# ironmanaudi/GNN-decode

Hardware: NVIDIA B200
Metric: decoded syndromes/sec (higher is better)
Workload: dtype f32

## Files before the change

### gnn_decode_b200/csrc/gd_lean.cu

```cuda
#include "gd_lean.cuh"
#include "gd_decode.cuh"
#include "gd_math.cuh"
#include "gd_options.cuh"
#include <algorithm>
#include <cmath>
#include <stddef.h>
#include <string.h>

namespace gd {

constexpr uint32_t kNone = 0xFFFFFFFFu;
constexpr int kMaxSlots = kLeanMaxSlots;
constexpr int kHdrBytes = 2048;
constexpr float kBudgetC = 1e-7f;
constexpr float kBudgetV = 1e-6f;
constexpr float kBudgetR = 4e-6f;

static_assert(sizeof(LeanHeader) <= kHdrBytes, "header");

struct LeanParams {
    const int* idx;
    const uint32_t* sgn;
    float* prob; float* logit; uint8_t* hard; uint32_t* hard_bits;
    LeanHeader* hdr;
    LeanCall* call;
    LeanCall* next_call;
    float* stash;
    LeanTrainHdr* train;
    const int* idx_src;
    const float4* ctab; const float4* rtab; const float4* vtab;
    const uint32_t* meta;
    long long B;
    int T, V, C, E, nw, vw, P;
    int v_lo, nv, part;
    int R, G, NCH;
    int ct_n, rt_n, vt_n;
    int train_vt_max;
    int off_me, off_ms, off_mi, off_var, off_ct, off_rt, off_vt, off_state;
};

__device__ __forceinline__ uint32_t lds_u32(uint32_t a) {
    uint32_t v;
    asm("ld.shared.u32 %0, [%1];" : "=r"(v) : "r"(a));
    return v;
}
__device__ __forceinline__ uint4 lds_u128(uint32_t a) {
    uint4 v;
    asm("ld.shared.v4.u32 {%0,%1,%2,%3}, [%4];" : "=r"(v.x), "=r"(v.y), "=r"(v.z), "=r"(v.w) : "r"(a));
    return v;
}
__device__ __forceinline__ uint2 lds_u64(uint32_t a) {
    uint2 v;
    asm("ld.shared.v2.u32 {%0,%1}, [%2];" : "=r"(v.x), "=r"(v.y) : "r"(a));
    return v;
}
__device__ __forceinline__ float4 lds_f128(uint32_t a) {
    float4 v;
    asm("ld.shared.v4.f32 {%0,%1,%2,%3}, [%4];" : "=f"(v.x), "=f"(v.y), "=f"(v.z), "=f"(v.w) : "r"(a));
    return v;
}
template <int OFF>
__device__ __forceinline__ float lds_state(uint32_t a) {
    float v;
    asm volatile("ld.shared.f32 %0, [%1+%2];" : "=f"(v) : "r"(a), "n"(OFF));
    return v;
}
template <int OFF>
__device__ __forceinline__ void sts_state(uint32_t a, float v) {
    asm volatile("st.shared.f32 [%0+%1], %2;" ::"r"(a), "n"(OFF), "f"(v));
}
__device__ __forceinline__ float lds_state_rt(uint32_t a) {
    float v;
    asm volatile("ld.shared.f32 %0, [%1];" : "=f"(v) : "r"(a));
    return v;
}
__device__ __forceinline__ void sts_state_rt(uint32_t a, float v) { asm volatile("st.shared.f32 [%0], %1;" ::"r"(a), "f"(v)); }
__device__ __forceinline__ void group_bar(int id, int nthreads) {
    asm volatile("bar.sync %0, %1;" ::"r"(id), "r"(nthreads) : "memory");
}

template <int STRIDE>
__device__ __forceinline__ float lean_cubic(uint32_t base, float w) {
    const float v = w + 12582912.0f;
    const float tau = w - (v - 12582912.0f);
    const float4 c = lds_f128((uint32_t)__float_as_int(v) * (uint32_t)STRIDE + base);
    return fmaf(fmaf(fmaf(c.w, tau, c.z), tau, c.y), tau, c.x);
}
template <int STRIDE>
__device__ __forceinline__ uint32_t lean_base(uint32_t piece0) {
    uint32_t b = piece0 - 0x4B400000u * (uint32_t)STRIDE;
    asm volatile("" : "+r"(b));
    return b;
}

__device__ __forceinline__ float lean_cubic_rt(uint32_t base, float w, uint32_t stride) {
    const float v = w + 12582912.0f;
    const float tau = w - (v - 12582912.0f);
    const float4 c = lds_f128((uint32_t)__float_as_int(v) * stride + base);
    return fmaf(fmaf(fmaf(c.w, tau, c.z), tau, c.y), tau, c.x);
}

struct LeanTabs {
    uint32_t vt_stride;
    uint32_t vt_base;
    uint32_t ct_base;
    float vt_inv_h, vt_off;
    float ct_inv_h, ct_off;
    float t0;
};

__device__ __forceinline__ float lean_vt(const LeanTabs& tb, float m) {
    return lean_cubic_rt(tb.vt_base, fmaf(m, tb.vt_inv_h, tb.vt_off), tb.vt_stride);
}
__device__ __forceinline__ float lean_ct(const LeanTabs& tb, float ext) {
    return lean_cubic<128>(tb.ct_base, fmaf(ext, tb.ct_inv_h, tb.ct_off));
}

template <int DEG, int NSIB, int CUR, int NXT, bool STASH>
__device__ __forceinline__ void lean_check(const uint4 eo, const uint4 so, uint32_t st_lane, const LeanTabs& tb, uint32_t sgn,
                                           float* stash_q, long long Bp) {
    const uint32_t eoa[4] = {eo.x, eo.y, eo.z, eo.w}, soa[4] = {so.x, so.y, so.z, so.w};
    float t[4], mo[4];
#pragma unroll
    for (int j = 0; j < 4; ++j) {
        t[j] = j < NSIB ? lean_vt(tb, lds_state<CUR>(st_lane + soa[j])) : (j < DEG ? tb.t0 : 0.f);
        mo[j] = j < DEG ? lds_state<CUR>(st_lane + eoa[j]) : 0.f;
    }
    const float a = t[0] + t[1], b = t[2] + t[3];
    const float ext[4] = {t[1] + b, t[0] + b, a + t[3], a + t[2]};
#pragma unroll
    for (int j = 0; j < DEG; ++j) {
        const float o = lean_ct(tb, ext[j]);
        const float mn = mo[j] + __uint_as_float(__float_as_uint(o) ^ sgn);
        sts_state<NXT>(st_lane + eoa[j], mn);
        if (STASH && stash_q) stash_q[(long long)(eoa[j] >> 8) * Bp] = mn;
    }
}

template <int CUR, bool STASH>
__device__ __forceinline__ void lean_iteration(const LeanParams& p, uint32_t me, uint32_t ms, uint32_t mi, uint32_t st_lane,
                                               const LeanTabs& tb, uint32_t mybits, float* stash_q) {
    constexpr int NXT = 128 - CUR;
#pragma unroll 1
    for (int k = 0; k < p.NCH; ++k) {
        const uint32_t kind = lds_u32(mi + 4u * k) & 63u;
        if (kind == 0) break;
        const uint4 eo = lds_u128(me + 16u * k), so = lds_u128(ms + 16u * k);
        const uint32_t sgn = (mybits >> k) << 31;
        switch (kind) {
#define GD_LEAN_CASE(D, S) case ((D) | ((S) << 3)): lean_check<D, S, CUR, NXT, STASH>(eo, so, st_lane, tb, sgn, stash_q, p.B); break;
            GD_LEAN_CASE(4, 4) GD_LEAN_CASE(4, 3) GD_LEAN_CASE(4, 2) GD_LEAN_CASE(4, 1) GD_LEAN_CASE(4, 0)
            GD_LEAN_CASE(3, 3) GD_LEAN_CASE(3, 2) GD_LEAN_CASE(3, 1) GD_LEAN_CASE(3, 0)
            GD_LEAN_CASE(2, 2) GD_LEAN_CASE(2, 1) GD_LEAN_CASE(2, 0)
            GD_LEAN_CASE(1, 1) GD_LEAN_CASE(1, 0)
#undef GD_LEAN_CASE
            default: break;
        }
    }
}

__device__ __forceinline__ void lean_deal(int n_slots, const int* counts, int* out4, int lane) {
        const int grid = (int)gridDim.x;
        int tl[2], nc[2];
        int total = 0;
#pragma unroll
        for (int h = 0; h < 2; ++h) {
            const int k = lane + 32 * h;
            tl[h] = k < n_slots ? (counts[k] + 31) >> 5 : 0;
            total += tl[h];
        }
        for (int o = 16; o > 0; o >>= 1) total += __shfl_xor_sync(0xffffffffu, total, o);
        int given = 0;
#pragma unroll
        for (int h = 0; h < 2; ++h) {
            nc[h] = tl[h] ? max(1, (int)((long long)grid * tl[h] / max(total, 1))) : 0;
            given += nc[h];
        }
        for (int o = 16; o > 0; o >>= 1) given += __shfl_xor_sync(0xffffffffu, given, o);
        for (int left = grid - given; left != 0; left += left > 0 ? -1 : 1) {
            float best = -3e38f;
            int who = -1;
#pragma unroll
            for (int h = 0; h < 2; ++h) {
                const bool can = left > 0 ? tl[h] > 0 : nc[h] > 1;
                const float load = left > 0 ? (float)tl[h] / (float)max(nc[h], 1) : -(float)tl[h] / (float)max(nc[h] - 1, 1);
                if (can && load > best) { best = load; who = lane + 32 * h; }
            }
            for (int o = 16; o > 0; o >>= 1) {
                const float ob = __shfl_xor_sync(0xffffffffu, best, o);
                const int ow = __shfl_xor_sync(0xffffffffu, who, o);
                if (ow >= 0 && (who < 0 || ob > best || (ob == best && ow < who))) { best = ob; who = ow; }
            }
            if (who < 0) break;
#pragma unroll
            for (int h = 0; h < 2; ++h)
                if (who == lane + 32 * h) nc[h] += left > 0 ? 1 : -1;
        }
        int my_slot = -1, my_part = 0, my_n = 1, my_tiles = 0, my_row0 = 0;
        int cta_acc = 0, row_acc = 0;
        for (int k = 0; k < n_slots; ++k) {
            const int src = k & 31, h = k >> 5;
            const int nk = __shfl_sync(0xffffffffu, h ? nc[1] : nc[0], src), tk = __shfl_sync(0xffffffffu, h ? tl[1] : tl[0], src);
            if (my_slot < 0 && nk > 0 && (int)blockIdx.x >= cta_acc && (int)blockIdx.x < cta_acc + nk) {
                my_slot = k; my_part = (int)blockIdx.x - cta_acc; my_n = nk; my_tiles = tk; my_row0 = row_acc;
            }
            cta_acc += nk;
            row_acc += counts[k];
        }
        if (lane == 0) {
            out4[0] = my_slot;
            out4[1] = my_slot >= 0 ? (int)((long long)my_part * my_tiles / my_n) : 0;
            out4[2] = my_slot >= 0 ? (int)((long long)(my_part + 1) * my_tiles / my_n) : 0;
            out4[3] = my_row0;
        }
}

template <bool STASH>
__global__ void __launch_bounds__(1024, 1) lean_decode_kernel(const LeanParams p) {
    extern __shared__ __align__(128) unsigned char smem[];
    __shared__ int tile_pre[4];
    pdl_enter();
    const LeanHeader* H = p.hdr;
    const int tid = threadIdx.x, lane = tid & 31, warp = tid >> 5;
    if (blockIdx.x == 0) {
        if (tid == 0) { p.next_call->overflow = 0; p.next_call->defer_count = 0; p.next_call->fmax_new = 0u; p.next_call->d2_new = 0u; p.next_call->d3_new = 0u; }
        if (tid < kMaxSlots) p.next_call->count[tid] = 0;
    }
    const int n_slots = H->n_slots;
    const float fmax = __uint_as_float(H->fmax_bits), f3max = __uint_as_float(H->f3max_bits);
    const bool overflow = p.call->overflow != 0;
    const int vt_n = H->vt_n_eff, vt_rep = vt_n > 0 ? (8 * p.vt_n) / vt_n : 0;
    const int vt_n_max = STASH ? p.train_vt_max : 8 * p.vt_n;
    bool ok = !overflow && n_slots <= kMaxSlots && vt_n >= p.vt_n && vt_n <= vt_n_max && __uint_as_float(H->err_c_bits) <= kBudgetC + 6e-8f * fmax &&
              __uint_as_float(H->err_r_bits) <= kBudgetR + 1e-7f * f3max && isfinite(fmax) && isfinite(f3max);
    const float gain = 6.0f * (float)p.T * __uint_as_float(H->d2max_bits) * __uint_as_float(H->d3max_bits);
    const float budget_v = gain > 400.0f ? 4e-4f / gain : kBudgetV;
    bool ok_v = isfinite(gain);
    float worst_v = 0.f;
    for (int k = 0; k < n_slots && k < kMaxSlots; ++k)
        if (p.call->count[k] != 0) worst_v = fmaxf(worst_v, __uint_as_float(H->err_v_bits[k]));
    ok_v = ok_v && worst_v <= budget_v;
    if (blockIdx.x == 0 && tid == 0 && ok && !overflow) {
        const int mult = max(1, H->vt_mult);
        if (!ok_v && vt_n < vt_n_max) { p.hdr->vt_mult = 2 * vt_n / p.vt_n; p.hdr->hash = 0ull; p.hdr->forced = 1; }
        else if (ok_v && mult > 1 && vt_n == mult * p.vt_n && worst_v * 32.0f < budget_v) p.hdr->vt_mult = mult / 2;
    }
    ok = ok && ok_v;
    if (STASH) ok = ok && p.call->defer_count == 0;
    if (STASH && blockIdx.x == 0 && tid < kMaxSlots) {
        if (tid == 0) {
            p.train->status = ok ? 1 : 0;
            p.train->old_count = ok ? 0 : -1;
            p.train->n_slots = n_slots;
            p.train->fmax_bits = H->fmax_bits;
            p.train->vt_n_eff = vt_n;
        }
        p.train->count[tid] = tid < n_slots ? p.call->count[tid] : 0;
        p.train->slot_bits[tid] = H->slot_bits[tid];
    }
    if (blockIdx.x == 0 && tid == 0) {
        if (overflow) {
            p.hdr->n_slots = 0;
            p.hdr->built_mask = 0ull;
            for (int k = 0; k < kMaxSlots; ++k) { p.hdr->slot_bits[k] = kNone; p.hdr->err_v_bits[k] = 0u; }
        } else {
            p.hdr->built_mask = n_slots >= 64 ? ~0ull : ((1ull << n_slots) - 1ull);
        }
        if (!ok) p.call->defer_count = -1;
    }
    if (!ok) return;
    if (n_slots == 0) return;
    if (STASH) {
        int* dst = reinterpret_cast<int*>(reinterpret_cast<float*>(p.train) + kLeanTrainTailFloats);
        for (long long i = (long long)blockIdx.x * blockDim.x + tid; i < p.B; i += (long long)gridDim.x * blockDim.x) dst[i] = p.idx_src[i];
    }

    if (warp == 0) lean_deal(n_slots, p.call->count, tile_pre, lane);
    __syncthreads();
    const int k = tile_pre[0], j_lo = tile_pre[1], j_hi = tile_pre[2];
    if (k < 0 || j_lo >= j_hi) return;
    {
        const uint4* src = reinterpret_cast<const uint4*>(p.meta);
        uint4* dst = reinterpret_cast<uint4*>(smem + p.off_me);
        const int n16 = (p.off_ct - p.off_me) >> 4;
        for (int i = tid; i < n16; i += blockDim.x) dst[i] = src[i];
        float4* ct = reinterpret_cast<float4*>(smem + p.off_ct);
        for (int i = tid; i < (p.ct_n + 2) * 8; i += blockDim.x) ct[i] = __ldg(p.ctab + (i >> 3));
        float4* rt = reinterpret_cast<float4*>(smem + p.off_rt);
        for (int i = tid; i < p.rt_n + 2; i += blockDim.x) rt[i] = __ldg(p.rtab + i);
        float4* vt = reinterpret_cast<float4*>(smem + p.off_vt);
        const float4* vsrc = p.vtab + (size_t)k * (8 * p.vt_n + 2);
        for (int i = tid; i < (vt_n + 2) * vt_rep; i += blockDim.x) vt[i] = __ldg(vsrc + i / vt_rep);
    }
    __syncthreads();
    const int grp = warp / p.R, r = warp - grp * p.R;
    const uint32_t s_base = (uint32_t)__cvta_generic_to_shared(smem);
    const uint32_t me = s_base + p.off_me + (uint32_t)(r * p.NCH) * 16u;
    const uint32_t ms = s_base + p.off_ms + (uint32_t)(r * p.NCH) * 16u;
    const uint32_t mi = s_base + p.off_mi + (uint32_t)(r * p.NCH) * 4u;
    const uint32_t st_lane = s_base + p.off_state + (uint32_t)grp * (uint32_t)p.E * 256u + (uint32_t)lane * 4u;
    const int bar_id = 1 + grp, bar_n = 32 * p.R;
    const float Rm = (float)p.T * (fmax * 1.02f + 1e-6f);
    LeanTabs tb;
    tb.vt_inv_h = 0.5f * (float)vt_n / Rm;
    tb.vt_off = Rm * tb.vt_inv_h - 0.5f;
    tb.ct_inv_h = (float)p.ct_n / 6.0f;
    tb.ct_off = 3.0f * tb.ct_inv_h - 0.5f;
    tb.ct_base = lean_base<128>(s_base + p.off_ct + 128u + (uint32_t)(lane & 7) * 16u);
    tb.vt_stride = 16u * (uint32_t)vt_rep;
    {
        uint32_t b = s_base + p.off_vt + tb.vt_stride + (uint32_t)(lane & (vt_rep - 1)) * 16u - 0x4B400000u * tb.vt_stride;
        asm volatile("" : "+r"(b));
        tb.vt_base = b;
    }
    const float rt_inv_h = 0.5f * (float)p.rt_n / Rm, rt_off = Rm * rt_inv_h - 0.5f;
    const uint32_t rt_base = lean_base<16>(s_base + p.off_rt + 16u);
    const int fin = (p.T & 1) * 128, oth = 128 - fin;

    {
        const float prior = __uint_as_float(H->slot_bits[k]);
        const int cnt = p.call->count[k];
        const int* rows = p.idx + tile_pre[3];
        tb.t0 = lean_vt(tb, 0.f);
        for (int j = j_lo + grp; j < j_hi; j += p.G) {
            const int li = j * 32 + lane;
            const bool live = li < cnt;
            const long long sg = live ? (long long)__ldg(rows + li) : 0;
            float* const stash_q = (STASH && live) ? p.stash + tile_pre[3] + li : nullptr;
            uint32_t mybits = 0;
            for (int q = 0; q < p.NCH; ++q) {
                const uint32_t info = lds_u32(mi + 4u * q);
                if ((info & 7u) == 0) break;
                const int c = (int)(info >> 8);
                const uint32_t wv = live ? __ldg(p.sgn + sg * p.nw + (c >> 5)) : 0u;
                mybits |= ((wv >> (c & 31)) & 1u) << q;
            }
            for (int q = 0; q < p.NCH; ++q) {
                const int deg = (int)(lds_u32(mi + 4u * q) & 7u);
                if (deg == 0) break;
                const uint4 eo = lds_u128(me + 16u * q);
                const float o = lean_ct(tb, (float)(deg - 1) * tb.t0);
                const float mv = __uint_as_float(__float_as_uint(o) ^ ((mybits >> q) << 31));
                const uint32_t eoa[4] = {eo.x, eo.y, eo.z, eo.w};
#pragma unroll
                for (int e = 0; e < 4; ++e)
                    if (e < deg) {
                        sts_state<128>(st_lane + eoa[e], mv);
                        if (STASH && stash_q) stash_q[(long long)(eoa[e] >> 8) * p.B] = mv;
                    }
            }
            group_bar(bar_id, bar_n);
            int it = 1;
            const long long EB = (long long)p.E * p.B;
            for (; it + 1 < p.T; it += 2) {
                lean_iteration<128, STASH>(p, me, ms, mi, st_lane, tb, mybits, stash_q ? stash_q + it * EB : nullptr);
                group_bar(bar_id, bar_n);
                lean_iteration<0, STASH>(p, me, ms, mi, st_lane, tb, mybits, stash_q ? stash_q + (it + 1) * EB : nullptr);
                group_bar(bar_id, bar_n);
            }
            if (it < p.T) {
                lean_iteration<128, STASH>(p, me, ms, mi, st_lane, tb, mybits, stash_q ? stash_q + it * EB : nullptr);
                group_bar(bar_id, bar_n);
            }
            const uint32_t st_grp = st_lane - (uint32_t)lane * 4u;
            for (int v = r; v < p.nv; v += p.R) {
                const uint2 ve = lds_u64(s_base + p.off_var + 8u * v);
                float acc = prior;
                if (ve.x != kNone) acc += lean_cubic<16>(rt_base, fminf(fmaxf(fmaf(lds_state_rt(st_lane + ve.x + fin), rt_inv_h, rt_off), -1.4f), (float)p.rt_n + 0.4f));
                if (ve.y != kNone) acc += lean_cubic<16>(rt_base, fminf(fmaxf(fmaf(lds_state_rt(st_lane + ve.y + fin), rt_inv_h, rt_off), -1.4f), (float)p.rt_n + 0.4f));
                const uint32_t q = (uint32_t)lane * (uint32_t)p.P + (uint32_t)v;
                sts_state_rt(st_grp + (q >> 5) * 256u + (q & 31u) * 4u + oth, acc);
            }
            group_bar(bar_id, bar_n);
            const int nvalid = min(32, cnt - j * 32);
            for (int s = r; s < nvalid; s += p.R) {
                const long long row = __shfl_sync(0xffffffffu, sg, s);
                for (int w = p.v_lo >> 5; w <= (p.v_lo + p.nv - 1) >> 5; ++w) {
                    const int v = w * 32 + lane, vl = v - p.v_lo;
                    const bool mine = vl >= 0 && vl < p.nv;
                    const uint32_t q = (uint32_t)s * (uint32_t)p.P + (uint32_t)(mine ? vl : 0);
                    const float lv = mine ? lds_state_rt(st_grp + (q >> 5) * 256u + (q & 31u) * 4u + oth) : 1.0f;
                    const float pr = sigmoid_neg(lv);
                    if (mine) {
                        if (p.prob) p.prob[row * p.V + v] = pr;
                        if (p.logit) p.logit[row * p.V + v] = lv;
                        if (p.hard) p.hard[row * p.V + v] = pr > 0.5f;
                    }
                    if (p.hard_bits) {
                        const uint32_t word = __ballot_sync(0xffffffffu, mine && pr > 0.5f);
                        if (lane == 0) { if (p.part) atomicOr(p.hard_bits + row * p.vw + w, word); else p.hard_bits[row * p.vw + w] = word; }
                    }
                }
            }
            group_bar(bar_id, bar_n);
        }
    }
}

struct MlpD {
    const float* w1; int w1s; const float* w1b; const float* b1; const float* w2; float b2; int h;
};
__device__ __forceinline__ void mlp_eval_warp(const MlpD& M, double prior, double x, int lane, double& f, double& df) {
    double sf = 0.0, sd = 0.0;
    for (int k = lane; k < M.h; k += 32) {
        const double a = (double)M.w1[k * M.w1s];
        double c = (double)M.b1[k];
        if (M.w1b) c += (double)M.w1b[k * M.w1s] * prior;
        const double z = a * x + c;
        double sp, sg;
        if (z > 20.0) { sp = z; sg = 1.0; }
        else {
            const double e = exp(-fabs(z));
            sp = fmax(z, 0.0) + log1p(e);
            sg = z >= 0.0 ? 1.0 / (1.0 + e) : e / (1.0 + e);
        }
        const double w2 = (double)M.w2[k];
        sf += w2 * sp;
        sd += w2 * a * sg;
    }
    for (int o = 16; o > 0; o >>= 1) {
        sf += __shfl_xor_sync(0xffffffffu, sf, o);
        sd += __shfl_xor_sync(0xffffffffu, sd, o);
    }
    f = sf + (double)M.b2;
    df = sd;
}
__device__ __forceinline__ void atomic_max_float_up(unsigned int* dst, double v) {
    const float f = __double2float_ru(fabs(v));
    atomicMax(dst, __float_as_uint(f));
}

constexpr int kChunk = 32;

__device__ void build_chunk(const MlpD& M, double prior, bool tanh_fold, double Rdom, int n, int i0, int n_int, float4* dst,
                            unsigned int* fmax_bits, unsigned int* dmax_bits, unsigned int* err_bits, double2* nodes ) {
    const int lane = threadIdx.x & 31, warp = threadIdx.x >> 5, nwarp = blockDim.x >> 5;
    const double h = 2.0 * Rdom / (double)n;
    for (int j = warp; j <= n_int; j += nwarp) {
        const double x = -Rdom + h * (double)(i0 - 1 + j);
        double f, df;
        mlp_eval_warp(M, prior, x, lane, f, df);
        if (lane == 0 && fmax_bits) atomic_max_float_up(fmax_bits, f);
        if (lane == 0 && dmax_bits) atomic_max_float_up(dmax_bits, df);
        if (tanh_fold) {
// ... 781 lines not shown
            for (int j = 0; j < 4; ++j) me[4 * i + j] = 0u, ms[4 * i + j] = kNone;
            mi[i] = 0u;
            if (k >= (int)own[r].size()) continue;
            const int c = own[r][k], b = g->h_chk_ptr[c], d = g->h_chk_ptr[c + 1] - b;
            int j = 0, nsib = 0;
            for (int pass = 0; pass < 2; ++pass)
                for (int q = 0; q < d; ++q) {
                    const int e = g->h_chk_edges[b + q];
                    const uint32_t sb = sibling(e);
                    if ((sb != kNone) != (pass == 0)) continue;
                    me[4 * i + j] = (uint32_t)loc[e] * 256u;
                    ms[4 * i + j] = sb;
                    nsib += sb != kNone;
                    ++j;
                }
            mi[i] = (uint32_t)d | ((uint32_t)nsib << 3) | ((uint32_t)c << 8);
        }
    for (int i = 0; i < sub->nv; ++i) {
        const int v = sub->v_lo + i, b = g->h_var_ptr[v], d = g->h_var_ptr[v + 1] - b;
        var[2 * i] = d > 0 ? (uint32_t)loc[g->h_var_edges[b]] * 256u : kNone;
        var[2 * i + 1] = d > 1 ? (uint32_t)loc[g->h_var_edges[b + 1]] * 256u : kNone;
    }
    if (cudaMalloc((void**)&m.dev, m.bytes) != cudaSuccess ||
        cudaMemcpy(m.dev, blob.data(), m.bytes, cudaMemcpyHostToDevice) != cudaSuccess) {
        if (m.dev) cudaFree(m.dev);
        m.dev = nullptr;
        cudaGetLastError();
    }
    ctx->metas.push_back(mp);
    return mp->dev ? mp : nullptr;
}

static bool lean_applicable(const gd_graph* g, const gd_model* m) {
    if (m->program != GD_PROG_V2_4 || m->flags != 0 || m->iters < 1 || m->iters > 32 || opt_on(OPT_NO_LEAN)) return false;
    if (g->max_var_deg > 2 || g->max_chk_deg > 4 || g->E >= (1 << 23) / 256) return false;
    return true;
}

static const int kLeanRts[] = {2048, 1024};
static int lean_rt_choice(gd_graph* g, const std::vector<const LeanSub*>& parts, int ct_n, int vt_n) {
    const int smem_max = g->max_smem_optin - 1024;
    int ri_all = 0;
    for (const LeanSub* sub : parts) {
        int g_cap[2] = {0, 0};
        for (int R = 1; R <= 32; ++R) {
            std::vector<std::vector<int>> own;
            int nch;
            double bal;
            assign_owners(g, sub, R, own, &nch, &bal);
            if (nch > 32 || nch == 0) continue;
            const int meta = align_up_i(align_up_i(2 * R * nch * 16 + R * nch * 4, 16) + sub->nv * 8, 16);
            for (int ri = 0; ri < 2; ++ri) {
                const int fixed = align_up_i(meta + (ct_n + 2) * 128 + (kLeanRts[ri] + 2) * 16 + (vt_n + 2) * 128, 128);
                g_cap[ri] = std::max(g_cap[ri], std::min((smem_max - fixed) / (sub->E * 256), std::min(32 / R, 15)));
            }
        }
        if (g_cap[1] < 1) return -1;
        if (!(g_cap[0] >= std::min(g_cap[1], 3) && g_cap[0] >= 1)) ri_all = 1;
    }
    return ri_all;
}

static bool lean_search(gd_graph* g, const LeanSub* sub, int tpc, int ri_fixed, LeanGeom* out) {
    const int E = sub->E, V = sub->nv;
    const int ct_n = (int)std::min<long long>(1024, std::max<long long>(32, opt_int(OPT_LEAN_CTAB_N, 128)));
    const int vt_n = (int)std::min<long long>(4096, std::max<long long>(64, opt_int(OPT_LEAN_VTAB_N, 512)));
    const int state = E * 256;
    const int smem_max = g->max_smem_optin - 1024;
    struct Cand { int R, G, NCH, rt_n; double score; };
    Cand best{0, 0, 0, 0, -1.0};
    const int* rts = kLeanRts;
    const long long force_R = opt_int(OPT_LEAN_R, 0), force_G = opt_int(OPT_LEAN_G, 0);
    const long long force_rt = opt_int(OPT_LEAN_RTAB_N, 0);
    std::vector<int> nchs(33, 0);
    std::vector<double> bals(33, 0.0);
    for (int R = 1; R <= 32; ++R) {
        std::vector<std::vector<int>> own;
        assign_owners(g, sub, R, own, &nchs[R], &bals[R]);
    }
    for (int R = 1; R <= 32; ++R) {
        if (force_R > 0 && R != force_R) continue;
        const int nch = nchs[R];
        const double bal = bals[R];
        if (nch > 32 || nch == 0) continue;
        const int meta = align_up_i(align_up_i(2 * R * nch * 16 + R * nch * 4, 16) + V * 8, 16);
        for (int ri = ri_fixed; ri <= ri_fixed; ++ri) {
            const int rt_n = force_rt > 0 ? (int)force_rt : rts[ri];
            const int fixed = align_up_i(meta + (ct_n + 2) * 128 + (rt_n + 2) * 16 + (vt_n + 2) * 128, 128);
            int G = (smem_max - fixed) / state;
            G = std::min(G, std::min(32 / R, 15));
            if (force_G > 0) G = G >= force_G ? (int)force_G : 0;
            if (G < 1) continue;
            const int warps = G * R;
            const double eff = (double)tpc / (double)(((tpc + G - 1) / G) * G);
            double score = (warps / (warps + 8.0)) * (G / (G + 0.8)) * std::sqrt(eff) * (0.4 + 0.6 * bal);
            if (score > best.score) best = Cand{R, G, nch, rt_n, score};
        }
    }
    if (best.R > 0 && force_R <= 0) {
        auto max_load = [&](int R) { return bals[R] > 0.0 ? (int)std::lround((double)E / ((double)R * bals[R])) : 0; };
        const int mx0 = max_load(best.R);
        for (int R = best.R + 1; R <= 32 && R * best.G <= 32; ++R) {
            if (nchs[R] == 0 || nchs[R] > best.NCH || max_load(R) > mx0) continue;
            const int meta = align_up_i(align_up_i(2 * R * nchs[R] * 16 + R * nchs[R] * 4, 16) + V * 8, 16);
            const int fixed = align_up_i(meta + (ct_n + 2) * 128 + (best.rt_n + 2) * 16 + (vt_n + 2) * 128, 128);
            if ((smem_max - fixed) / state < best.G) continue;
            best.R = R; best.NCH = nchs[R];
        }
    }
    out->valid = true;
    out->R = best.R; out->G = best.G; out->NCH = best.NCH; out->rt_n = best.rt_n;
    out->ct_n = ct_n; out->vt_n = vt_n;
    return true;
}

static bool lean_fill(gd_graph* g, const LeanSub* sub, const gd_model* m, int64_t B, const LeanGeom& best, const LeanMeta* meta, LeanPlan* out) {
    const int E = sub->E, V = g->V, ct_n = best.ct_n, vt_n = best.vt_n, state = E * 256;
    const int smem_max = g->max_smem_optin;
    LeanParams& p = out->p;
    memset(&p, 0, sizeof(p));
    p.B = B; p.T = m->iters; p.V = V; p.C = g->C; p.E = E;
    p.nw = (g->C + 31) / 32; p.vw = (V + 31) / 32; p.P = sub->nv | 1;
    p.v_lo = sub->v_lo; p.nv = sub->nv; p.part = sub->id >= 0 ? 1 : 0;
    p.R = best.R; p.G = best.G; p.NCH = meta->NCH;
    p.ct_n = ct_n; p.rt_n = best.rt_n; p.vt_n = vt_n;
    p.meta = meta->dev;
    p.off_me = 0; p.off_ms = meta->off_ms; p.off_mi = meta->off_mi; p.off_var = meta->off_var;
    p.off_ct = (int)meta->bytes;
    p.off_rt = p.off_ct + (ct_n + 2) * 128;
    p.off_vt = p.off_rt + (best.rt_n + 2) * 16;
    p.off_state = align_up_i(p.off_vt + (vt_n + 2) * 128, 128);
    out->smem = p.off_state + best.G * state;
    out->threads = 32 * best.G * best.R;
    out->n_tiles = (int)((B + 31) / 32);
    out->grid = g->sm_count;
    out->meta = meta;
    return out->smem <= smem_max - 1024;
}

static bool lean_plan(gd_graph* g, const gd_model* m, int64_t B, std::vector<LeanPlan>* out, bool whole_only = false) {
    out->clear();
    if (!lean_applicable(g, m)) return false;
    const std::vector<LeanSub*>& subs = lean_subs(g);
    const int ct_n = (int)std::min<long long>(1024, std::max<long long>(32, opt_int(OPT_LEAN_CTAB_N, 128)));
    const int vt_n = (int)std::min<long long>(4096, std::max<long long>(64, opt_int(OPT_LEAN_VTAB_N, 512)));
    const int tpc = (int)std::min<long long>(64, std::max<long long>(1, ((B + 31) / 32 + g->sm_count - 1) / g->sm_count));
    LeanCtx* ctx = static_cast<LeanCtx*>(g->lean_ctx);
    int mode = -2, ri = -1;
    {
        std::lock_guard<std::mutex> lk(g->mu);
        if (ctx->mode_epoch == opt_epoch()) { mode = ctx->mode[whole_only ? 1 : 0]; ri = ctx->mode_ri[whole_only ? 1 : 0]; }
    }
    if (mode == -2) {
        int modes[2], ris[2];
        const int ri_whole = (subs[0]->nv | 1) <= subs[0]->E ? lean_rt_choice(g, {subs[0]}, ct_n, vt_n) : -1;
        std::vector<const LeanSub*> comps(subs.begin() + 1, subs.end());
        bool comps_ok = !comps.empty();
        for (const LeanSub* c : comps) comps_ok = comps_ok && (c->nv | 1) <= c->E;
        const int ri_comps = comps_ok ? lean_rt_choice(g, comps, ct_n, vt_n) : -1;
        const long long want = opt_int(OPT_LEAN_PARTS, -1);
        modes[1] = ri_whole >= 0 ? 0 : -1; ris[1] = ri_whole;
        if (ri_comps >= 0 && (ri_whole < 0 || want == 1) && want != 0) { modes[0] = 1; ris[0] = ri_comps; }
        else { modes[0] = modes[1]; ris[0] = ri_whole; }
        std::lock_guard<std::mutex> lk(g->mu);
        ctx->mode_epoch = opt_epoch();
        for (int i = 0; i < 2; ++i) { ctx->mode[i] = modes[i]; ctx->mode_ri[i] = ris[i]; }
        mode = modes[whole_only ? 1 : 0]; ri = ris[whole_only ? 1 : 0];
    }
    if (mode < 0) return false;
    const size_t first = mode == 0 ? 0 : 1, last = mode == 0 ? 1 : subs.size();
    for (size_t si = first; si < last; ++si) {
        const LeanSub* sub = subs[si];
        LeanGeom geom;
        {
            std::lock_guard<std::mutex> lk(g->mu);
            if (!ctx->geoms.empty() && ctx->geoms[0].opt_epoch != opt_epoch()) ctx->geoms.clear();
            for (const LeanGeom& q : ctx->geoms)
                if (q.tpc == tpc && q.sub == sub->id) geom = q;
        }
        if (!geom.valid) {
            if (!lean_search(g, sub, tpc, ri, &geom)) return false;
            geom.opt_epoch = opt_epoch();
            geom.tpc = tpc;
            geom.sub = sub->id;
            std::lock_guard<std::mutex> lk(g->mu);
            if (ctx->geoms.size() >= 128) ctx->geoms.clear();
            ctx->geoms.push_back(geom);
        }
        if (geom.R == 0) return false;
        const LeanMeta* meta = get_meta(g, sub, geom.R);
        if (!meta) return false;
        LeanPlan pl;
        if (!lean_fill(g, sub, m, B, geom, meta, &pl)) return false;
        pl.n_parts = (int)(last - first);
        out->push_back(pl);
    }
    return !out->empty();
}

bool lean_launch_info(const gd_graph* g, const gd_model* model, int64_t B, gd_launch_info* out) {
    std::vector<LeanPlan> pls;
    if (!lean_plan(const_cast<gd_graph*>(g), model, B, &pls)) return false;
    const LeanPlan& pl = pls[0];
    out->tile = 32 * pl.p.G; out->threads = pl.threads; out->grid = pl.grid; out->smem_bytes = pl.smem;
    out->resident = 1; out->n_tiles = (int)pls.size() * ((pl.n_tiles + pl.p.G - 1) / pl.p.G);
    return true;
}

template <typename P>
static cudaError_t pdl_launch(void (*kern)(const P), dim3 grid, dim3 block, size_t smem, cudaStream_t st, const P& params) {
    return pdl_launch_on(!opt_on(OPT_NO_PDL), kern, grid, block, smem, st, params);
}

static cudaMemPool_t lean_pool(gd_graph* g) {
    std::lock_guard<std::mutex> lk(g->mu);
    if (!g->lean_ctx) g->lean_ctx = new LeanCtx();
    LeanCtx* ctx = static_cast<LeanCtx*>(g->lean_ctx);
    if (!ctx->pool) {
        cudaMemPoolProps props;
        memset(&props, 0, sizeof(props));
        props.allocType = cudaMemAllocationTypePinned;
        props.handleTypes = cudaMemHandleTypeNone;
        props.location.type = cudaMemLocationTypeDevice;
        props.location.id = g->device;
        if (cudaMemPoolCreate(&ctx->pool, &props) != cudaSuccess) {
            ctx->pool = nullptr;
            cudaGetLastError();
            return nullptr;
        }
        unsigned long long keep = ~0ull;
        cudaMemPoolSetAttribute(ctx->pool, cudaMemPoolAttrReleaseThreshold, &keep);
    }
    return ctx->pool;
}

static bool lean_bwd_geom(gd_graph* g, const LeanParams& fp, LeanBwdGeom* out) {
    LeanCtx* ctx = static_cast<LeanCtx*>(g->lean_ctx);
    const int tpc = (int)std::min<long long>(64, std::max<long long>(1, ((fp.B + 31) / 32 + g->sm_count - 1) / g->sm_count));
    {
        std::lock_guard<std::mutex> lk(g->mu);
        if (!ctx->bwd.empty() && ctx->bwd[0].opt_epoch != opt_epoch()) ctx->bwd.clear();
        for (const LeanBwdGeom& c : ctx->bwd)
            if (c.valid && c.tpc == tpc && c.ct_n == fp.ct_n && c.rt_n == fp.rt_n && c.vt_n == fp.vt_n) {
                *out = c;
                return c.R > 0;
            }
    }
    const int E = (int)g->E, ct_n = fp.ct_n, rt_n = fp.rt_n, vt_n = fp.vt_n;
    const int smem_max = g->max_smem_optin - 1024;
    auto fixed_bytes = [&](int meta, int n) {
        return align_up_i(meta + (ct_n + 2 + rt_n + 2 + n + 2) * 16 + 16 * (ct_n + 3 + rt_n + 3 + n + 3), 128);
    };
    LeanBwdGeom b;
    double best = -1.0;
    std::vector<int> nchs(33, 0), mxs(33, 0), metas(33, 0);
    auto take = [&](int R, int G) {
        b.R = R; b.G = G;
        b.vt_max = vt_n;
        for (int mult = 2; mult <= 4; mult *= 2)
            if (fixed_bytes(metas[R], mult * vt_n) + 3 * E * 128 <= smem_max) b.vt_max = mult * vt_n;
    };
    for (int R = 1; R <= 32; ++R) {
        std::vector<std::vector<int>> own;
        int nch;
        double bal;
        assign_owners(g, lean_subs(g)[0], R, own, &nch, &bal);
        if (nch == 0 || nch > 32) continue;
        const int meta = align_up_i(align_up_i(2 * R * nch * 16 + R * nch * 4, 16) + g->V * 8, 16);
        nchs[R] = nch; metas[R] = meta; mxs[R] = bal > 0.0 ? (int)std::lround((double)E / ((double)R * bal)) : 0;
        int G = (smem_max - fixed_bytes(meta, vt_n)) / (3 * E * 128);
        G = std::min(G, std::min(32 / R, 15));
        if (G < 1) continue;
        G = std::min(G, tpc);
        const int warps = G * R;
        const double eff = (double)tpc / (double)(((tpc + G - 1) / G) * G);
        const double score = (warps / (warps + 8.0)) * (G / (G + 0.8)) * std::sqrt(eff) * (0.4 + 0.6 * bal);
        if (score > best) { best = score; take(R, G); }
    }
    if (b.R > 0) {
        const int r0 = b.R;
        for (int R = r0 + 1; R <= 32 && R * b.G <= 32; ++R) {
            if (nchs[R] == 0 || nchs[R] > nchs[r0] || mxs[R] > mxs[r0]) continue;
            if ((smem_max - fixed_bytes(metas[R], vt_n)) / (3 * E * 128) < b.G) continue;
            take(R, b.G);
        }
    }
    b.ct_n = ct_n; b.rt_n = rt_n; b.vt_n = vt_n; b.tpc = tpc; b.opt_epoch = opt_epoch(); b.valid = true;
    {
        std::lock_guard<std::mutex> lk(g->mu);
// ... 51 lines not shown
        hit->ct_n = p.ct_n; hit->rt_n = p.rt_n; hit->vt_n = p.vt_n;
    }
    hit->last_use = ++ctx->tick;
    return hit;
}

int lean_decode(gd_graph* g, const gd_model* model, const float* weights_dev, const float* x_dev, const float* prior_dev,
                const uint32_t* synd_dev, float* prob_dev, float* logit_dev, uint8_t* hard_dev, uint32_t* hard_bits_dev,
                int64_t B, cudaStream_t st, float* stash_dev) {
    std::vector<LeanPlan> pls;
    if (!lean_plan(g, model, B, &pls, stash_dev != nullptr)) return -1;
    cudaMemPool_t pool = lean_pool(g);
    if (!pool) return -1;
    LeanCtx* ctx = static_cast<LeanCtx*>(g->lean_ctx);
    std::lock_guard<std::mutex> enq(ctx->enq);
    LeanParams& p = pls[0].p;
    LeanEntry* ent = lean_entry(g, ctx, p, model, weights_dev, st);
    if (!ent) return -1;
    const int N = g->N;
    size_t off = 0;
    auto take = [&](size_t bytes) { const size_t o = off; off = (off + bytes + 255) & ~(size_t)255; return o; };
    const size_t o_slot = take((size_t)B * 2), o_pos = take((size_t)B * 4), o_idx = take((size_t)B * 4);
    const size_t o_sgn = take(x_dev ? (size_t)B * p.nw * 4 : 0);
    const size_t o_defer = take((size_t)B * 4), o_x = take(x_dev ? 0 : (size_t)B * N * 4);
    unsigned char* ws = nullptr;
    GD_CUDA(cudaMallocFromPoolAsync((void**)&ws, off, pool, st));
    LeanHeader* hdr = reinterpret_cast<LeanHeader*>(ent->dev);
    LeanCall* call = &hdr->calls[ent->calls & 1];
    LeanCall* next_call = &hdr->calls[(ent->calls + 1) & 1];
    ++ent->calls;
    float4* ctab = reinterpret_cast<float4*>(ent->dev + ent->o_ct);
    float4* rtab = reinterpret_cast<float4*>(ent->dev + ent->o_rt);
    float4* vtab = reinterpret_cast<float4*>(ent->dev + ent->o_vt);
    int rc = GD_OK;
    cudaError_t e = cudaSuccess;
    {
        PrepParams pp;
        memset(&pp, 0, sizeof(pp));
        pp.x = x_dev; pp.weights = weights_dev; pp.hdr = hdr; pp.call = call;
        pp.sgn_out = reinterpret_cast<uint32_t*>(ws + o_sgn);
        pp.prior_in = prior_dev; pp.slot = reinterpret_cast<short*>(ws + o_slot); pp.pos = reinterpret_cast<int*>(ws + o_pos);
        pp.defer_idx = reinterpret_cast<int*>(ws + o_defer);
        pp.B = B; pp.V = g->V; pp.C = g->C; pp.N = N; pp.nw = p.nw;
        pp.n_w = (int)gd_weights_size(model); pp.T = model->iters; pp.ct_n = p.ct_n; pp.rt_n = p.rt_n; pp.vt_n = p.vt_n;
        pp.rows_per_block = x_dev ? 64 : kPrepRows;
        while ((B + pp.rows_per_block - 1) / pp.rows_per_block > (1 << 18) && pp.rows_per_block < kPrepRows) pp.rows_per_block *= 2;
        const long long blocks = (B + pp.rows_per_block - 1) / pp.rows_per_block;
        GD_CHECK_ARG(blocks < (1ll << 30), "gd_decode_fwd: batch too large for the table kernel's prep pass");
        pp.hid = model->hidden;
        pp.keep_mult = stash_dev ? 1 : 0;
        pp.fm_blocks = (p.ct_n + 3 + kD3Points + 7) / 8;
        e = pdl_launch(lean_prep_kernel, dim3((unsigned int)(1 + pp.fm_blocks + blocks)), dim3(256), 0, st, pp);
    }
    if (e == cudaSuccess) {
        TabParams tp;
        memset(&tp, 0, sizeof(tp));
        tp.weights = weights_dev; tp.hdr = hdr; tp.call = call; tp.ctab = ctab; tp.rtab = rtab; tp.vtab = vtab;
        tp.slot = reinterpret_cast<const short*>(ws + o_slot); tp.pos = reinterpret_cast<const int*>(ws + o_pos);
        tp.idx = reinterpret_cast<int*>(ws + o_idx); tp.B = B;
        tp.hid = model->hidden; tp.T = model->iters; tp.ct_n = p.ct_n; tp.rt_n = p.rt_n; tp.vt_n = p.vt_n;
        tp.ct_blocks = (p.ct_n + 2 + kChunk - 1) / kChunk;
        tp.rt_blocks = (p.rt_n + 2 + kChunk - 1) / kChunk;
        tp.vt_chunks = 2 * g->sm_count;
        tp.scatter_blocks = (int)std::max<long long>(1, std::min<long long>((B + 1023) / 1024, (long long)g->sm_count * 4));
        e = pdl_launch(lean_tables_kernel, dim3(tp.scatter_blocks + tp.ct_blocks + tp.rt_blocks + tp.vt_chunks), dim3(256), 0, st, tp);
    }
    if (e == cudaSuccess && pls.size() > 1 && hard_bits_dev)
        e = cudaMemsetAsync(hard_bits_dev, 0, (size_t)B * p.vw * sizeof(uint32_t), st);
    for (size_t pi = 0; pi < pls.size() && e == cudaSuccess; ++pi) {
        LeanPlan& pl = pls[pi];
        LeanParams& q = pl.p;
        q.idx = reinterpret_cast<const int*>(ws + o_idx);
        q.sgn = x_dev ? reinterpret_cast<const uint32_t*>(ws + o_sgn) : synd_dev;
        q.prob = prob_dev; q.logit = logit_dev; q.hard = hard_dev; q.hard_bits = hard_bits_dev;
        q.hdr = hdr; q.call = call; q.next_call = next_call;
        q.ctab = ctab; q.rtab = rtab; q.vtab = vtab;
        q.stash = stash_dev;
        q.train = stash_dev ? lean_train_hdr(stash_dev, g, model, B) : nullptr;
        if (stash_dev) {
            LeanBwdGeom bg;
            q.train_vt_max = lean_bwd_geom(g, q, &bg) ? bg.vt_max : 0;
        }
        q.idx_src = q.idx;
        auto kern = stash_dev ? lean_decode_kernel<true> : lean_decode_kernel<false>;
        e = cudaFuncSetAttribute(kern, cudaFuncAttributeMaxDynamicSharedMemorySize, pl.smem);
        if (e == cudaSuccess) e = pdl_launch(kern, dim3(pl.grid), dim3(pl.threads), (size_t)pl.smem, st, q);
    }
    cudaEventRecord(ent->ev, st);
    const float* x_for_deferred = x_dev;
    if (e == cudaSuccess && !x_dev) {
        float* xw = reinterpret_cast<float*>(ws + o_x);
        lean_unpack_kernel<<<g->sm_count * 4, 256, 0, st>>>(prior_dev, synd_dev, call, reinterpret_cast<const int*>(ws + o_defer), xw,
                                                            B, g->V, g->C, p.nw);
        e = cudaGetLastError();
        x_for_deferred = xw;
    }
    if (e == cudaSuccess) {
        const DeferList dl{stash_dev ? &lean_train_hdr(stash_dev, g, model, B)->old_count : &call->defer_count,
                           reinterpret_cast<const int*>(ws + o_defer)};
        rc = decode_fwd_deferred(g, model, weights_dev, x_for_deferred, prob_dev, logit_dev, hard_dev, hard_bits_dev, B, st, dl, stash_dev);
    }
    cudaError_t ef = cudaFreeAsync(ws, st);
    if (rc != GD_OK) return rc;
    GD_CUDA(e);
    GD_CUDA(ef);
    return GD_OK;
}

int packed_via_unpack(gd_graph* g, const float* prior_dev, const uint32_t* synd_dev, int64_t B, cudaStream_t st,
                      int (*run)(void* ctx, const float* x_dev), void* ctx) {
    cudaMemPool_t pool = lean_pool(g);
    if (!pool) {
        set_error("gd_decode_packed_fwd: no memory pool on device %d", g->device);
        return GD_ERR_CUDA;
    }
    float* xw = nullptr;
    GD_CUDA(cudaMallocFromPoolAsync((void**)&xw, (size_t)B * g->N * sizeof(float), pool, st));
    lean_unpack_kernel<<<g->sm_count * 4, 256, 0, st>>>(prior_dev, synd_dev, nullptr, nullptr, xw, B, g->V, g->C, (g->C + 31) / 32);
    cudaError_t e = cudaGetLastError();
    int rc = e == cudaSuccess ? run(ctx, xw) : GD_OK;
    cudaError_t ef = cudaFreeAsync(xw, st);
    if (rc != GD_OK) return rc;
    GD_CUDA(e);
    GD_CUDA(ef);
    return GD_OK;
}

int64_t lean_bwd_bins_floats(const gd_graph* g, const gd_model* model) {
    if (!lean_applicable(g, model)) return 0;
    const int ct_n = (int)std::min<long long>(1024, std::max<long long>(32, opt_int(OPT_LEAN_CTAB_N, 128)));
    const int vt_n = (int)std::min<long long>(4096, std::max<long long>(64, opt_int(OPT_LEAN_VTAB_N, 512)));
    return 2 * 2 * ((int64_t)(ct_n + 3) + (2048 + 3) + (int64_t)kMaxSlots * (4 * vt_n + 3));
}

int lean_backward(gd_graph* g, const gd_model* model, const float* weights_dev, const float* x_dev, const float* stash_dev,
                  const float* grad_logit_dev, float* grad_weights_dev, float* bins_dev, int accumulate, int64_t B, cudaStream_t st) {
    std::vector<LeanPlan> fwds;
    if (!lean_plan(g, model, B, &fwds, true)) return -1;
    const LeanPlan& fwd = fwds[0];
    LeanCtx* ctx = static_cast<LeanCtx*>(g->lean_ctx);
    std::lock_guard<std::mutex> enq(ctx->enq);
    LeanEntry* ent = nullptr;
    for (LeanEntry* e : ctx->entries)
        if (e->st == st && e->w == weights_dev && e->T == model->iters && e->hid == model->hidden && e->ct_n == fwd.p.ct_n &&
            e->rt_n == fwd.p.rt_n && e->vt_n == fwd.p.vt_n)
            ent = e;
    if (!ent) {
        set_error("gd_decode_bwd: no table set of a matching gd_decode_fwd_train on this stream (call the forward first)");
        return GD_ERR_INVALID;
    }
    LeanBwdParams p;
    memset(&p, 0, sizeof(p));
    const int E = (int)g->E, ct_n = fwd.p.ct_n, rt_n = fwd.p.rt_n, vt_n = fwd.p.vt_n;
    LeanBwdGeom bg;
    if (!lean_bwd_geom(g, fwd.p, &bg)) return -1;
    const int bestR = bg.R, bestG = bg.G;
    const LeanMeta* meta = get_meta(g, lean_subs(g)[0], bestR);
    if (!meta) return -1;
    const LeanTrainHdr* hdr = lean_train_hdr(const_cast<float*>(stash_dev), g, model, B);
    p.x = x_dev; p.stash = stash_dev; p.train = hdr; p.grad_logit = grad_logit_dev;
    p.ctab = reinterpret_cast<const float4*>(ent->dev + ent->o_ct);
    p.rtab = reinterpret_cast<const float4*>(ent->dev + ent->o_rt);
    p.vtab = reinterpret_cast<const float4*>(ent->dev + ent->o_vt);
    p.meta = meta->dev; p.bins = reinterpret_cast<long long*>(bins_dev);
    p.B = B; p.T = model->iters; p.V = g->V; p.C = g->C; p.E = E; p.N = g->N; p.R = bestR; p.G = bestG; p.NCH = meta->NCH;
    p.ct_n = ct_n; p.rt_n = rt_n; p.vt_n = vt_n;
    p.off_me = 0; p.off_ms = meta->off_ms; p.off_mi = meta->off_mi; p.off_var = meta->off_var;
    p.off_ct = (int)meta->bytes;
// ... 34 lines not shown
```

Before: 389.9 million.

## Keep check-to-variable messages in registers and store pre-transformed variable messages

Check-node messages now live in a per-thread register array sized by the chunk count NCH, which becomes a template parameter. Shared memory holds the variable-table-transformed values instead of raw messages, so each sibling read no longer needs its own table lookup. Only the last iteration writes raw messages back. To make room in the register file, launch bounds and the planner's group count are cut for larger NCH, and plans with NCH above 8 are now rejected. This trades fewer threads per CTA and more kernel instantiations for fewer shared-memory loads and table evaluations per iteration.

```diff
diff --git a/gnn_decode_b200/csrc/gd_lean.cu b/gnn_decode_b200/csrc/gd_lean.cu
--- a/gnn_decode_b200/csrc/gd_lean.cu
+++ b/gnn_decode_b200/csrc/gd_lean.cu
@@ -17,6 +17,9 @@
 constexpr float kBudgetR = 4e-6f;
 
 static_assert(sizeof(LeanHeader) <= kHdrBytes, "header");
+
+constexpr int kLeanMaxNCH = 8;
+__host__ __device__ constexpr int lean_max_threads(int nch) { return nch <= 4 ? 1024 : nch <= 7 ? 640 : 512; }
 
 struct LeanParams {
     const int* idx;
@@ -41,12 +44,12 @@
 
 __device__ __forceinline__ uint32_t lds_u32(uint32_t a) {
     uint32_t v;
-    asm("ld.shared.u32 %0, [%1];" : "=r"(v) : "r"(a));
+    asm volatile("ld.shared.u32 %0, [%1];" : "=r"(v) : "r"(a));
     return v;
 }
 __device__ __forceinline__ uint4 lds_u128(uint32_t a) {
     uint4 v;
-    asm("ld.shared.v4.u32 {%0,%1,%2,%3}, [%4];" : "=r"(v.x), "=r"(v.y), "=r"(v.z), "=r"(v.w) : "r"(a));
+    asm volatile("ld.shared.v4.u32 {%0,%1,%2,%3}, [%4];" : "=r"(v.x), "=r"(v.y), "=r"(v.z), "=r"(v.w) : "r"(a));
     return v;
 }
 __device__ __forceinline__ uint2 lds_u64(uint32_t a) {
@@ -116,39 +119,37 @@
     return lean_cubic<128>(tb.ct_base, fmaf(ext, tb.ct_inv_h, tb.ct_off));
 }
 
-template <int DEG, int NSIB, int CUR, int NXT, bool STASH>
+template <int DEG, int NSIB, int CUR, int NXT, bool STASH, bool LAST>
 __device__ __forceinline__ void lean_check(const uint4 eo, const uint4 so, uint32_t st_lane, const LeanTabs& tb, uint32_t sgn,
-                                           float* stash_q, long long Bp) {
+                                           float (&m)[4], float* stash_q, long long Bp) {
     const uint32_t eoa[4] = {eo.x, eo.y, eo.z, eo.w}, soa[4] = {so.x, so.y, so.z, so.w};
-    float t[4], mo[4];
-#pragma unroll
-    for (int j = 0; j < 4; ++j) {
-        t[j] = j < NSIB ? lean_vt(tb, lds_state<CUR>(st_lane + soa[j])) : (j < DEG ? tb.t0 : 0.f);
-        mo[j] = j < DEG ? lds_state<CUR>(st_lane + eoa[j]) : 0.f;
-    }
+    float t[4];
+#pragma unroll
+    for (int j = 0; j < 4; ++j) t[j] = j < NSIB ? lds_state<CUR>(st_lane + soa[j]) : (j < DEG ? tb.t0 : 0.f);
     const float a = t[0] + t[1], b = t[2] + t[3];
     const float ext[4] = {t[1] + b, t[0] + b, a + t[3], a + t[2]};
 #pragma unroll
     for (int j = 0; j < DEG; ++j) {
         const float o = lean_ct(tb, ext[j]);
-        const float mn = mo[j] + __uint_as_float(__float_as_uint(o) ^ sgn);
-        sts_state<NXT>(st_lane + eoa[j], mn);
-        if (STASH && stash_q) stash_q[(long long)(eoa[j] >> 8) * Bp] = mn;
-    }
-}
-
-template <int CUR, bool STASH>
+        m[j] = m[j] + __uint_as_float(__float_as_uint(o) ^ sgn);
+        if (LAST) sts_state<NXT>(st_lane + eoa[j], m[j]);
+        else if (j < NSIB) sts_state<NXT>(st_lane + eoa[j], lean_vt(tb, m[j]));
+        if (STASH && stash_q) stash_q[(long long)(eoa[j] >> 8) * Bp] = m[j];
+    }
+}
+
+template <int NCH, int CUR, bool STASH, bool LAST>
 __device__ __forceinline__ void lean_iteration(const LeanParams& p, uint32_t me, uint32_t ms, uint32_t mi, uint32_t st_lane,
-                                               const LeanTabs& tb, uint32_t mybits, float* stash_q) {
+                                               const LeanTabs& tb, uint32_t mybits, float (&m)[NCH][4], float* stash_q) {
     constexpr int NXT = 128 - CUR;
-#pragma unroll 1
-    for (int k = 0; k < p.NCH; ++k) {
+#pragma unroll
+    for (int k = 0; k < NCH; ++k) {
         const uint32_t kind = lds_u32(mi + 4u * k) & 63u;
         if (kind == 0) break;
         const uint4 eo = lds_u128(me + 16u * k), so = lds_u128(ms + 16u * k);
         const uint32_t sgn = (mybits >> k) << 31;
         switch (kind) {
-#define GD_LEAN_CASE(D, S) case ((D) | ((S) << 3)): lean_check<D, S, CUR, NXT, STASH>(eo, so, st_lane, tb, sgn, stash_q, p.B); break;
+#define GD_LEAN_CASE(D, S) case ((D) | ((S) << 3)): lean_check<D, S, CUR, NXT, STASH, LAST>(eo, so, st_lane, tb, sgn, m[k], stash_q, p.B); break;
             GD_LEAN_CASE(4, 4) GD_LEAN_CASE(4, 3) GD_LEAN_CASE(4, 2) GD_LEAN_CASE(4, 1) GD_LEAN_CASE(4, 0)
             GD_LEAN_CASE(3, 3) GD_LEAN_CASE(3, 2) GD_LEAN_CASE(3, 1) GD_LEAN_CASE(3, 0)
             GD_LEAN_CASE(2, 2) GD_LEAN_CASE(2, 1) GD_LEAN_CASE(2, 0)
@@ -215,8 +216,8 @@
         }
 }
 
-template <bool STASH>
-__global__ void __launch_bounds__(1024, 1) lean_decode_kernel(const LeanParams p) {
+template <bool STASH, int NCH>
+__global__ void __launch_bounds__(lean_max_threads(NCH), 1) lean_decode_kernel(const LeanParams p) {
     extern __shared__ __align__(128) unsigned char smem[];
     __shared__ int tile_pre[4];
     pdl_enter();
@@ -328,38 +329,51 @@
             const long long sg = live ? (long long)__ldg(rows + li) : 0;
             float* const stash_q = (STASH && live) ? p.stash + tile_pre[3] + li : nullptr;
             uint32_t mybits = 0;
-            for (int q = 0; q < p.NCH; ++q) {
+#pragma unroll
+            for (int q = 0; q < NCH; ++q) {
                 const uint32_t info = lds_u32(mi + 4u * q);
                 if ((info & 7u) == 0) break;
                 const int c = (int)(info >> 8);
                 const uint32_t wv = live ? __ldg(p.sgn + sg * p.nw + (c >> 5)) : 0u;
                 mybits |= ((wv >> (c & 31)) & 1u) << q;
             }
-            for (int q = 0; q < p.NCH; ++q) {
-                const int deg = (int)(lds_u32(mi + 4u * q) & 7u);
+            float m[NCH][4] = {};
+#pragma unroll
+            for (int q = 0; q < NCH; ++q) {
+                const uint32_t info = lds_u32(mi + 4u * q);
+                const int deg = (int)(info & 7u), nsib = (int)((info >> 3) & 7u);
                 if (deg == 0) break;
-                const uint4 eo = lds_u128(me + 16u * q);
                 const float o = lean_ct(tb, (float)(deg - 1) * tb.t0);
                 const float mv = __uint_as_float(__float_as_uint(o) ^ ((mybits >> q) << 31));
+#pragma unroll
+                for (int e = 0; e < 4; ++e) m[q][e] = mv;
+                const uint4 eo = lds_u128(me + 16u * q);
                 const uint32_t eoa[4] = {eo.x, eo.y, eo.z, eo.w};
+                const float tv = (p.T > 1 && nsib > 0) ? lean_vt(tb, mv) : 0.f;
 #pragma unroll
                 for (int e = 0; e < 4; ++e)
                     if (e < deg) {
-                        sts_state<128>(st_lane + eoa[e], mv);
+                        if (p.T == 1) sts_state<128>(st_lane + eoa[e], mv);
+                        else if (e < nsib) sts_state<128>(st_lane + eoa[e], tv);
                         if (STASH && stash_q) stash_q[(long long)(eoa[e] >> 8) * p.B] = mv;
                     }
             }
             group_bar(bar_id, bar_n);
             int it = 1;
             const long long EB = (long long)p.E * p.B;
-            for (; it + 1 < p.T; it += 2) {
-                lean_iteration<128, STASH>(p, me, ms, mi, st_lane, tb, mybits, stash_q ? stash_q + it * EB : nullptr);
+            for (; it + 2 < p.T; it += 2) {
+                lean_iteration<NCH, 128, STASH, false>(p, me, ms, mi, st_lane, tb, mybits, m, stash_q ? stash_q + it * EB : nullptr);
                 group_bar(bar_id, bar_n);
-                lean_iteration<0, STASH>(p, me, ms, mi, st_lane, tb, mybits, stash_q ? stash_q + (it + 1) * EB : nullptr);
+                lean_iteration<NCH, 0, STASH, false>(p, me, ms, mi, st_lane, tb, mybits, m, stash_q ? stash_q + (it + 1) * EB : nullptr);
                 group_bar(bar_id, bar_n);
             }
-            if (it < p.T) {
-                lean_iteration<128, STASH>(p, me, ms, mi, st_lane, tb, mybits, stash_q ? stash_q + it * EB : nullptr);
+            if (it + 1 < p.T) {
+                lean_iteration<NCH, 128, STASH, false>(p, me, ms, mi, st_lane, tb, mybits, m, stash_q ? stash_q + it * EB : nullptr);
+                group_bar(bar_id, bar_n);
+                lean_iteration<NCH, 0, STASH, true>(p, me, ms, mi, st_lane, tb, mybits, m, stash_q ? stash_q + (it + 1) * EB : nullptr);
+                group_bar(bar_id, bar_n);
+            } else if (it < p.T) {
+                lean_iteration<NCH, 128, STASH, true>(p, me, ms, mi, st_lane, tb, mybits, m, stash_q ? stash_q + it * EB : nullptr);
                 group_bar(bar_id, bar_n);
             }
             const uint32_t st_grp = st_lane - (uint32_t)lane * 4u;
@@ -1307,13 +1321,13 @@
         if (force_R > 0 && R != force_R) continue;
         const int nch = nchs[R];
         const double bal = bals[R];
-        if (nch > 32 || nch == 0) continue;
+        if (nch > kLeanMaxNCH || nch == 0) continue;
         const int meta = align_up_i(align_up_i(2 * R * nch * 16 + R * nch * 4, 16) + V * 8, 16);
         for (int ri = ri_fixed; ri <= ri_fixed; ++ri) {
             const int rt_n = force_rt > 0 ? (int)force_rt : rts[ri];
             const int fixed = align_up_i(meta + (ct_n + 2) * 128 + (rt_n + 2) * 16 + (vt_n + 2) * 128, 128);
             int G = (smem_max - fixed) / state;
-            G = std::min(G, std::min(32 / R, 15));
+            G = std::min(G, std::min(lean_max_threads(nch) / (32 * R), 15));
             if (force_G > 0) G = G >= force_G ? (int)force_G : 0;
             if (G < 1) continue;
             const int warps = G * R;
@@ -1326,7 +1340,7 @@
         auto max_load = [&](int R) { return bals[R] > 0.0 ? (int)std::lround((double)E / ((double)R * bals[R])) : 0; };
         const int mx0 = max_load(best.R);
         for (int R = best.R + 1; R <= 32 && R * best.G <= 32; ++R) {
-            if (nchs[R] == 0 || nchs[R] > best.NCH || max_load(R) > mx0) continue;
+            if (nchs[R] == 0 || nchs[R] > best.NCH || max_load(R) > mx0 || 32 * R * best.G > lean_max_threads(nchs[R])) continue;
             const int meta = align_up_i(align_up_i(2 * R * nchs[R] * 16 + R * nchs[R] * 4, 16) + V * 8, 16);
             const int fixed = align_up_i(meta + (ct_n + 2) * 128 + (best.rt_n + 2) * 16 + (vt_n + 2) * 128, 128);
             if ((smem_max - fixed) / state < best.G) continue;
@@ -1430,6 +1444,12 @@
     out->tile = 32 * pl.p.G; out->threads = pl.threads; out->grid = pl.grid; out->smem_bytes = pl.smem;
     out->resident = 1; out->n_tiles = (int)pls.size() * ((pl.n_tiles + pl.p.G - 1) / pl.p.G);
     return true;
+}
+
+template <bool STASH, int N = 1>
+static void (*lean_decode_fn(int nch))(const LeanParams) {
+    if constexpr (N > kLeanMaxNCH) return nullptr;
+    else return nch == N ? lean_decode_kernel<STASH, N> : lean_decode_fn<STASH, N + 1>(nch);
 }
 
 template <typename P>
@@ -1647,8 +1667,8 @@
             q.train_vt_max = lean_bwd_geom(g, q, &bg) ? bg.vt_max : 0;
         }
         q.idx_src = q.idx;
-        auto kern = stash_dev ? lean_decode_kernel<true> : lean_decode_kernel<false>;
-        e = cudaFuncSetAttribute(kern, cudaFuncAttributeMaxDynamicSharedMemorySize, pl.smem);
+        auto kern = stash_dev ? lean_decode_fn<true>(q.NCH) : lean_decode_fn<false>(q.NCH);
+        e = kern ? cudaFuncSetAttribute(kern, cudaFuncAttributeMaxDynamicSharedMemorySize, pl.smem) : cudaErrorInvalidDeviceFunction;
         if (e == cudaSuccess) e = pdl_launch(kern, dim3(pl.grid), dim3(pl.threads), (size_t)pl.smem, st, q);
     }
     cudaEventRecord(ent->ev, st);
```

Result: slower. 339.3 million (median of 6 runs) (-13.0%).
